# zju3dv/NeuralRecon-W

Measured on AMD Instinct MI355X. Metric: ray-samples/sec (train step) at 1024 rays x 128 samples, higher is better.
Workload: dtype f16; 1 GPU; brandenburg_gate config (BASELINE.json configs[1]): 1024 rays/GPU x (64 coarse + 64 fine) samples, SDF 8x256 + colour 4x256 + bg NeRF 8x256, 4 outside samples, up_sample_steps 2, render+loss+backward+allreduce+clip+Adam; rays_per_gpu=1024, samples_per_ray=128, global_rays=1024, parallelism=dp1, world_size=1, submission=eager, streams=2, skipped_steps=0

## Files before the change

neuralrecon-w_amd/csrc/ncw_color.hip:

```cpp
#include <stdlib.h>

#include "ncw_mlp.h"


namespace NCW_NS {

NCW_DEV void build_aux2(CVec<1>& aux, const float (&x)[3], const float (&nrm)[3], int lane) {
    const int h = lane >> 5;
#pragma unroll
    for (int r = 0; r < 16; ++r) {
        float v = 0.f;
        if (ncw_feat_of(r, 0) < 6) {
            const int f = ncw_feat_of(r, 0) + 4 * h;
            v = f == 0 ? x[0] : f == 1 ? x[1] : f == 2 ? x[2] : f == 3 ? nrm[0] : f == 4 ? nrm[1] : f == 5 ? nrm[2] : 0.f;
        }
        aux.v[0][r] = v;
    }
}

template <bool SPLIT, int RB_IN, int RB_OUT, int K_REAL, int SLOT, class P>
NCW_DEV void mma_stream_split(CVec<RB_OUT>& acc, const Act<P, RB_IN>& in, WRing& ring, const typename P::welem* __restrict__ w_hi,
                              const void* w_lo, int self_bytes, const void* w_next, int next_bytes, int lane) {
    typedef typename P::welem WE;
    if (SPLIT) {
// ... 19 lines not shown
        for (int r = 0; r < 16; ++r) yv[r] = ncw_relu(acc.v[rb][r]);
        if (st) stash_store_block(st, tile, RB, rb, yv, lane);
        to_act_block_hl<P, RB>(act, act_lo, rb, yv);
    }
}

template <int RB_IN, int RB_OUT, int K_REAL, int SLOT, class P>
NCW_DEV void mma_stream_split3(CVec<RB_OUT>& acc, const Act<P, RB_IN>& in, const Act<P, RB_IN>& in_lo, WRing& ring,
                               const typename P::welem* __restrict__ w_hi, const void* w_lo, int self_bytes, const void* w_next,
                               int next_bytes, int lane) {
    typedef typename P::welem WE;
    mma_stream2<RB_IN, RB_OUT, K_REAL, SLOT>(acc, in, in_lo, ring, w_hi, w_lo, self_bytes, lane);
    mma_stream<RB_IN, RB_OUT, K_REAL, SLOT>(acc, in, ring, (const WE*)w_lo, w_next, next_bytes, lane);
}

template <class P, int RBF, int RBH, int RBC, bool WIDE = false>
struct ColShapes {
    static constexpr int OCC = (RBF >= 16 || WIDE) ? 1 : 2;
    static constexpr int SLOT = RingSlot<RBC, OCC>::bytes;
    static constexpr int FCB_F = ncw_first_chunk_bytes<P, RBF, 32 * RBF, RBF, SLOT>();
    static constexpr int FCB_E0 = ncw_first_chunk_bytes<P, RBF + 3, 32 * RBF + 96, RBH, SLOT>();
    static constexpr int FCB_E = ncw_first_chunk_bytes<P, RBH, 32 * RBH, RBH, SLOT>();
    static constexpr int FCB_L0 = ncw_first_chunk_bytes<P, RBH + 1, 32 * RBH + 6, RBC, SLOT>();
    static constexpr int FCB_L = ncw_first_chunk_bytes<P, RBC, 32 * RBC, RBC, SLOT>();
    static constexpr int FCB_LAST = ncw_first_chunk_bytes<P, RBC, 32 * RBC, 1, SLOT>();
    static constexpr int FCB_TLAST = ncw_first_chunk_bytes<P, 1, 3, RBC, SLOT>();
    static constexpr int FCB_TL0 = ncw_first_chunk_bytes<P, RBC, 32 * RBC, RBH + 1, SLOT>();
    static constexpr int FCB_TE0 = ncw_first_chunk_bytes<P, RBH, 32 * RBH, RBF + 3, SLOT>();
};

template <class P, int RBF, int RBH, int RBC, int SPLIT, bool TRAIN>
NCW_DEV void color_fwd_body(const NcwColorNet& net, const NcwPoints& src, int64_t n, const float* __restrict__ normals,
                            const float* __restrict__ a, const void* __restrict__ feat_stash, float* __restrict__ rgb,
                            const NcwColorStash& st) {
    typedef typename P::welem WE;
    typedef typename P::selem SE;
    auto stp = [](void* p) -> SE* { return TRAIN ? (SE*)p : nullptr; };
    typedef ColShapes<P, RBF, RBH, RBC, SPLIT == 2> SH;
    constexpr bool AS = SPLIT == 2;
    NCW_RING_DECL(SH::SLOT);
    const int lane = ncw_lane();
    ring_prologue(ring, net.w_f, SH::FCB_F);
    int64_t tile, p, ray;
    bool valid;
    tile_setup(n, tile, p, valid, lane);
    float xs[3];
    load_point(src, p, xs, ray);
    const float dir[3] = {src.rays_d[ray * 3 + 0], src.rays_d[ray * 3 + 1], src.rays_d[ray * 3 + 2]};
    const float nrm[3] = {normals[p * 3 + 0], normals[p * 3 + 1], normals[p * 3 + 2]};

    Act<P, 3> aux1a;
    {
        CVec<3> aux1;
        build_aux1<Fast<P>::v>(aux1, dir, a + ray * net.n_a, net.n_a, lane);
        if (TRAIN) stash_store<3>((SE*)st.aux1, tile, aux1, lane);
        to_act(aux1a, aux1);
        if (st.aux_bias != nullptr) ncw_act_zero3(aux1a);
    }
    Act<P, 1> aux2a, aux2lo;
    {
        CVec<1> aux2;
        build_aux2(aux2, xs, nrm, lane);
        if (TRAIN) stash_store<1>((SE*)st.aux2, tile, aux2, lane);
        if constexpr (SPLIT != 0) {
#pragma unroll
            for (int t = 0; t < 2; ++t) ncw_split8(aux2.v[0], t, aux2a.f[t], aux2lo.f[t]);
        } else {
            to_act(aux2a, aux2);
        }
    }
    Act<P, RBF + 3> cat1;
    Act<P, (AS ? RBF + 3 : 1)> cat1_lo;
    {
        Act<P, RBF> fin;
#pragma unroll
        for (int rb = 0; rb < RBF; ++rb) {
            f32x16 v;
            stash_load_block(v, (const SE*)feat_stash, tile, RBF, rb, lane);
            to_act_block<RBF>(fin, rb, v);
        }
        CVec<RBF> f;
        load_bias(f, net.b_f, lane);
        mma_stream_split<(SPLIT != 0), RBF, RBF, 32 * RBF, SH::SLOT>(f, fin, ring, (const WE*)net.w_f, net.w_f_lo, SH::FCB_F, net.w_e[0],
                                                                SH::FCB_E0, lane);
        if (TRAIN) stash_store<RBF>((SE*)st.f, tile, f, lane);
        if constexpr (AS) {
            Act<P, RBF> fa, fl;
#pragma unroll
            for (int rb = 0; rb < RBF; ++rb) to_act_block_hl<P, RBF>(fa, fl, rb, f.v[rb]);
            act_concat<RBF, 3>(cat1, fa, aux1a);
            Act<P, 3> z3;
            ncw_act_zero3(z3);
            act_concat<RBF, 3>(cat1_lo, fl, z3);
        } else {
            Act<P, RBF> fa;
            to_act(fa, f);
            act_concat<RBF, 3>(cat1, fa, aux1a);
        }
    }
    Act<P, RBH> ea;
    Act<P, (AS ? RBH : 1)> ea_lo;
    {
        CVec<RBH> e;
        load_bias(e, net.b_e[0], lane);
        if (st.aux_bias != nullptr) ncw_add_ray_bias<RBH>(e, st.aux_bias + ray * (32 * RBH), lane);
        const void* wn = net.n_head > 1 ? net.w_e[1] : net.w_l[0];
        const int nb = net.n_head > 1 ? SH::FCB_E : SH::FCB_L0;
// ... 51 lines not shown
                mma_stream<RBH + 1, RBC, 32 * RBH + 6, SH::SLOT>(x, cat2, ring, (const WE*)net.w_l[0], net.w_l[1], nxt, lane);
            }
        } else {
            mma_stream_split<false, RBH + 1, RBC, 32 * RBH + 6, SH::SLOT>(x, cat2, ring, (const WE*)net.w_l[0], net.w_l_lo[0], SH::FCB_L0,
                                                                          net.w_l[1], 1 == last ? SH::FCB_LAST : SH::FCB_L, lane);
        }
        if constexpr (AS) relu_epilogue_hl<P, RBC>(xa, xa_lo, x, stp(st.x[0]), tile, lane);
        else relu_epilogue<P, RBC>(xa, x, stp(st.x[0]), tile, lane);
    }
    for (int l = 1; l < last; ++l) {
        load_bias(x, net.b_l[l], lane);
        if constexpr (AS) {
            mma_stream_split3<RBC, RBC, 32 * RBC, SH::SLOT>(x, xa, xa_lo, ring, (const WE*)net.w_l[l], net.w_l_lo[l], SH::FCB_L,
                                                            net.w_l[l + 1], l + 1 == last ? SH::FCB_LAST : SH::FCB_L, lane);
            relu_epilogue_hl<P, RBC>(xa, xa_lo, x, stp(st.x[l]), tile, lane);
        } else {
            mma_stream_split<(SPLIT != 0), RBC, RBC, 32 * RBC, SH::SLOT>(x, xa, ring, (const WE*)net.w_l[l], net.w_l_lo[l], SH::FCB_L,
                                                                    net.w_l[l + 1], l + 1 == last ? SH::FCB_LAST : SH::FCB_L, lane);
            relu_epilogue<P, RBC>(xa, x, stp(st.x[l]), tile, lane);
        }
    }
    CVec<1> o;
    load_bias(o, net.b_l[last], lane);
    if constexpr (AS)
        mma_stream_split3<RBC, 1, 32 * RBC, SH::SLOT>(o, xa, xa_lo, ring, (const WE*)net.w_l[last], net.w_l_lo[last], SH::FCB_LAST,
                                                      nullptr, 0, lane);
    else
        mma_stream_split<(SPLIT != 0), RBC, 1, 32 * RBC, SH::SLOT>(o, xa, ring, (const WE*)net.w_l[last], net.w_l_lo[last], SH::FCB_LAST,
                                                              nullptr, 0, lane);
    if (valid && lane < 32) {
        rgb[p * 3 + 0] = sigmoidf_<Fast<P>::v>(o.v[0][0]);
        rgb[p * 3 + 1] = sigmoidf_<Fast<P>::v>(o.v[0][1]);
        rgb[p * 3 + 2] = sigmoidf_<Fast<P>::v>(o.v[0][2]);
    }
}

template <class P, int RBF, int RBH, int RBC, int SPLIT = 0>
__global__ __launch_bounds__(64 * NCW_WG_WAVES, ((RBF >= 16 || SPLIT == 2) ? 1 : 2)) void color_fwd_kernel(NcwColorNet net, NcwPoints src, int64_t n,
                                                                      const float* __restrict__ normals,
                                                                      const float* __restrict__ a,
                                                                      const void* __restrict__ feat_stash,
                                                                      float* __restrict__ rgb, NcwColorStash st) {
    color_fwd_body<P, RBF, RBH, RBC, SPLIT, true>(net, src, n, normals, a, feat_stash, rgb, st);
}
template <class P, int RBF, int RBH, int RBC, int SPLIT = 0>
__global__ __launch_bounds__(64 * NCW_WG_WAVES, ((RBF >= 16 || SPLIT == 2) ? 1 : 2)) void color_render_kernel(NcwColorNet net, NcwPoints src, int64_t n,
                                                                         const float* __restrict__ normals,
                                                                         const float* __restrict__ a,
                                                                         const void* __restrict__ feat_stash,
                                                                         float* __restrict__ rgb, NcwColorStash st) {
    color_fwd_body<P, RBF, RBH, RBC, SPLIT, false>(net, src, n, normals, a, feat_stash, rgb, st);
}

template <class P, int RBF, int RBH, int RBC>
__global__ __launch_bounds__(64 * NCW_WG_WAVES, (RBF >= 16 ? 1 : 2)) void color_bwd_kernel(NcwColorNet net, NcwPoints src, int64_t n,
                                                                      const float* __restrict__ rgb,
                                                                      const float* __restrict__ d_rgb,
                                                                      float* __restrict__ d_grad, float* __restrict__ d_a,
                                                                      float* __restrict__ d_a_rows,
                                                                      void* __restrict__ dfeat_stash, NcwColorStash st) {
    typedef typename P::welem WE;
    typedef typename P::selem SE;
    typedef ColShapes<P, RBF, RBH, RBC> SH;
    NCW_RING_DECL(SH::SLOT);
    const int lane = ncw_lane();
    const int last = net.n_lin - 1;
    ring_prologue(ring, net.wt_l[last], SH::FCB_TLAST);
    int64_t tile, p, ray;
    bool valid;
    tile_setup(n, tile, p, valid, lane);
    ray = (src.mode == 0) ? p : p / src.per_ray;
    const float vm = valid ? 1.f : 0.f;

    CVec<1> zo;
    cvec_zero(zo);
    if (lane < 32) {
#pragma unroll
        for (int c = 0; c < 3; ++c) {
            const float y = rgb[p * 3 + c];
            zo.v[0][c] = d_rgb[p * 3 + c] * y * (1.f - y) * vm;
        }
    }
    stash_store<1>((SE*)st.zo, tile, zo, lane);
    Act<P, 1> zoa;
    to_act(zoa, zo);
    CVec<RBC> u;
    cvec_zero(u);
    mma_stream<1, RBC, 3, SH::SLOT>(u, zoa, ring, (const WE*)net.wt_l[last], net.wt_l[last - 1],
                                    last - 1 == 0 ? SH::FCB_TL0 : SH::FCB_L, lane);
    Act<P, RBC> za;
    for (int l = last - 1; l >= 1; --l) {
        relu_backward<P, RBC>(za, u, (const SE*)st.x[l], (SE*)st.zx[l], tile, lane);
        cvec_zero(u);
        mma_stream<RBC, RBC, 32 * RBC, SH::SLOT>(u, za, ring, (const WE*)net.wt_l[l], net.wt_l[l - 1],
                                                  l - 1 == 0 ? SH::FCB_TL0 : SH::FCB_L, lane);
    }
    CVec<RBH> ue;
    {
        relu_backward<P, RBC>(za, u, (const SE*)st.x[0], (SE*)st.zx[0], tile, lane);
        CVec<RBH + 1> q;
        cvec_zero(q);
        const void* wn = net.n_head > 1 ? net.wt_e[net.n_head - 1] : net.wt_e[0];
        const int nb = net.n_head > 1 ? SH::FCB_E : SH::FCB_TE0;
        mma_stream<RBC, RBH + 1, 32 * RBC, SH::SLOT>(q, za, ring, (const WE*)net.wt_l[0], wn, nb, lane);
#pragma unroll
        for (int rb = 0; rb < RBH; ++rb) ue.v[rb] = q.v[rb];
        if (valid) {
            if (lane < 32) d_grad[p * 3 + 0] += q.v[RBH][3];
            else {
                d_grad[p * 3 + 1] += q.v[RBH][0];
                d_grad[p * 3 + 2] += q.v[RBH][1];
            }
        }
    }
    Act<P, RBH> zea;
    for (int i = net.n_head - 1; i >= 1; --i) {
        relu_backward<P, RBH>(zea, ue, (const SE*)st.e[i], (SE*)st.ze[i], tile, lane);
        cvec_zero(ue);
        mma_stream<RBH, RBH, 32 * RBH, SH::SLOT>(ue, zea, ring, (const WE*)net.wt_e[i], net.wt_e[i - 1],
                                                  i - 1 == 0 ? SH::FCB_TE0 : SH::FCB_E, lane);
    }
    {
        relu_backward<P, RBH>(zea, ue, (const SE*)st.e[0], (SE*)st.ze[0], tile, lane);
        CVec<RBF + 3> q;
        cvec_zero(q);
        mma_stream<RBH, RBF + 3, 32 * RBH, SH::SLOT>(q, zea, ring, (const WE*)net.wt_e[0], net.wt_f, SH::FCB_F, lane);
        CVec<3> qa;
        qa.v[0] = q.v[RBF]; qa.v[1] = q.v[RBF + 1]; qa.v[2] = q.v[RBF + 2];
        accumulate_d_a(qa, d_a, ray, net.n_a, valid, lane, d_a_rows, p);
        CVec<RBF> zf;
#pragma unroll
        for (int rb = 0; rb < RBF; ++rb) zf.v[rb] = q.v[rb];
        stash_store<RBF>((SE*)st.zf, tile, zf, lane);
        Act<P, RBF> zfa;
        to_act(zfa, zf);
        CVec<RBF> df;
        cvec_zero(df);
        mma_stream<RBF, RBF, 32 * RBF, SH::SLOT>(df, zfa, ring, (const WE*)net.wt_f, nullptr, 0, lane);
        stash_store<RBF>((SE*)dfeat_stash, tile, df, lane);
    }
}

}
using namespace NCW_NS;

static bool color_ok(const NcwColorNet* net) {
    return net && net->n_head >= 1 && net->n_head <= 4 && net->n_lin >= 2 && net->n_lin <= 8 && net->n_a >= 0 &&
           net->n_a <= 69;
}

#define NCW_COLOR_DISPATCH(KERNEL, ...)                                                                          \
    do {                                                                                                         \
        const int key = net->rbf * 10000 + net->rbh * 100 + net->rbc;                                            \
        if (prec == NCW_PREC_F32) {                                                                              \
            if (key == 20102) NCW_LAUNCH_TILES((KERNEL<PrecF32, 2, 1, 2>), n, st, __VA_ARGS__);                  \
            else if (key == 20408) NCW_LAUNCH_TILES((KERNEL<PrecF32, 2, 4, 8>), n, st, __VA_ARGS__);             \
            else if (key == 80408) NCW_LAUNCH_TILES((KERNEL<PrecF32, 8, 4, 8>), n, st, __VA_ARGS__);             \
            else if (key == 160408) NCW_LAUNCH_TILES((KERNEL<PrecF32, 16, 4, 8>), n, st, __VA_ARGS__);           \
            else return NCW_E_UNSUPPORTED;                                                                       \
        } else {                                                                                                 \
            if (key == 20102) NCW_LAUNCH_TILES((KERNEL<PrecBF16, 2, 1, 2>), n, st, __VA_ARGS__);                 \
            else if (key == 20408) NCW_LAUNCH_TILES((KERNEL<PrecBF16, 2, 4, 8>), n, st, __VA_ARGS__);            \
            else if (key == 80408) NCW_LAUNCH_TILES((KERNEL<PrecBF16, 8, 4, 8>), n, st, __VA_ARGS__);            \
            else if (key == 160408) NCW_LAUNCH_TILES((KERNEL<PrecBF16, 16, 4, 8>), n, st, __VA_ARGS__);          \
            else return NCW_E_UNSUPPORTED;                                                                       \
        }                                                                                                        \
    } while (0)

#ifndef NCW_HALF_F16
extern "C" int ncw_color_fwd_f16(const NcwColorNet*, int, const NcwPoints*, int64_t, const float*, const float*, const void*, float*,
                                 const NcwColorStash*, void*);
extern "C" int ncw_color_bwd_f16(const NcwColorNet*, int, const NcwPoints*, int64_t, const float*, const float*, float*, float*, float*,
                                 void*, const NcwColorStash*, void*);
#endif

extern "C" int NCW_FN(ncw_color_fwd)(const NcwColorNet* net, int prec, const NcwPoints* pts, int64_t n, const float* normals,
                                     const float* a, const void* feat_stash, float* rgb, const NcwColorStash* stash,
                                     void* stream) {
    NCW_FORWARD_F16(prec, ncw_color_fwd_f16(net, NCW_PREC_BF16, pts, n, normals, a, feat_stash, rgb, stash, stream));
    if (!color_ok(net) || !pts || !stash || n < 0 || (prec != NCW_PREC_F32 && prec != NCW_PREC_BF16)) return NCW_E_BADARG;
    if (pts->mode == 4) return NCW_E_UNSUPPORTED;
    if (n == 0) return 0;
    hipStream_t st = (hipStream_t)stream;
    const bool render = stash->aux1 == nullptr;
    if (net->w_f_lo != nullptr) {
        if (prec == NCW_PREC_F32) return NCW_E_BADARG;
        const int key = net->rbf * 10000 + net->rbh * 100 + net->rbc;
        for (int i = 0; i < net->n_head; ++i) if (net->w_e_lo[i] == nullptr) return NCW_E_BADARG;
        for (int l = 0; l < net->n_lin; ++l) if (net->w_l_lo[l] == nullptr) return NCW_E_BADARG;
#define NCW_COLOR_SPLIT_DISPATCH(KERNEL, S)                                                                                               \
        do {                                                                                                                                    \
// ... 38 lines not shown
```

neuralrecon-w_amd/csrc/ncw_common.h:

```cpp
#pragma once
#include <hip/hip_runtime.h>
#include <stdint.h>
#include <type_traits>

#ifdef NCW_HALF_F16
typedef _Float16 ncw_h16;
#define NCW_MFMA_H __builtin_amdgcn_mfma_f32_32x32x16_f16
#define NCW_FN(name) name##_f16
#define NCW_NS ncw_h_f16
#else
typedef __bf16 ncw_h16;
#define NCW_MFMA_H __builtin_amdgcn_mfma_f32_32x32x16_bf16
#define NCW_FN(name) name
#define NCW_NS ncw_h_bf16
#endif
typedef ncw_h16 bf16x8 __attribute__((ext_vector_type(8)));
typedef ncw_h16 bf16x4 __attribute__((ext_vector_type(4)));
typedef float f32x16 __attribute__((ext_vector_type(16)));
typedef float f32x4 __attribute__((ext_vector_type(4)));

#define NCW_PREC_F32 0
#define NCW_PREC_BF16 1
#define NCW_PREC_F16 2
#ifdef NCW_HALF_F16
// ... 125 lines not shown
NCW_HD constexpr int ncw_chunk_units(int rb_stride, int n_units, int slot_bytes) {
    int g = slot_bytes / ncw_unit_bytes<P>(rb_stride);
    if (g < 1) g = 1;
    return g < n_units ? g : n_units;
}
template <class P, int RB_IN, int K_REAL, int RB_STRIDE, int SLOT>
NCW_HD constexpr int ncw_first_chunk_bytes() {
    return ncw_chunk_units<P>(RB_STRIDE, ncw_nb_used(RB_IN, K_REAL) * UnitsPerBlock<P>::v, SLOT) *
           ncw_unit_bytes<P>(RB_STRIDE);
}

NCW_DEV void ring_prologue(WRing& ring, const void* w_first, int first_bytes) {
    ring.cur = 0;
    ring_issue(ring.slot(0), w_first, first_bytes);
}

template <int RB_IN>
NCW_DEV float unit_b(const Act<PrecF32, RB_IN>& in, int rb, int sub) { return in.v[rb][sub]; }
template <int RB_IN>
NCW_DEV bf16x8 unit_b(const Act<PrecBF16, RB_IN>& in, int rb, int sub) { return in.f[2 * rb + sub]; }

NCW_DEV f32x16 unit_mfma(float a, float b, const f32x16& c) { return __builtin_amdgcn_mfma_f32_32x32x2f32(a, b, c, 0, 0, 0); }
NCW_DEV f32x16 unit_mfma(const bf16x8& a, const bf16x8& b, const f32x16& c) {
    return NCW_MFMA_H(a, b, c, 0, 0, 0);
}

template <class P>
NCW_HD constexpr int ncw_unit_first_feature(int rb, int sub) {
    return (P::id == NCW_PREC_F32) ? 32 * rb + ncw_feat_of(sub, 0) : 16 * (2 * rb + sub);
}

template <class P, int RB_IN_>
struct ActB {
    static constexpr int RB_IN = RB_IN_;
    const Act<P, RB_IN_>& a;
    NCW_DEV explicit ActB(const Act<P, RB_IN_>& a_) : a(a_) {}
    NCW_DEV void prepare(int) {}
    NCW_DEV auto b(int rb, int sub) const { return unit_b<RB_IN_>(a, rb, sub); }
};

template <class P, int RA, int RG>
struct CatB {
    static constexpr int RB_IN = RA + RG;
    const Act<P, RA>& a;
    const Act<P, RG>& g;
    NCW_DEV CatB(const Act<P, RA>& a_, const Act<P, RG>& g_) : a(a_), g(g_) {}
    NCW_DEV void prepare(int) {}
    NCW_DEV auto b(int rb, int sub) const {
        return rb < RA ? unit_b<RA>(a, rb < RA ? rb : 0, sub) : unit_b<RG>(g, rb >= RA ? rb - RA : 0, sub);
    }
};

struct NoB2 {};
template <int RB_OUT, int K_REAL, int SLOT, int RB_STRIDE, class P, class BP, bool PIPE = (SLOT != 32768) && (RB_OUT <= 8), class BP2 = NoB2>
NCW_DEV void mma_stream_b(CVec<RB_OUT>& acc, BP& bp, WRing& ring, const typename P::welem* __restrict__ wp,
                          const void* w_next, int next_bytes, int lane, BP2* bp2 = nullptr) {
    constexpr int RB_IN = BP::RB_IN;
    constexpr int UPB = UnitsPerBlock<P>::v;
    constexpr int NU = ncw_nb_used(RB_IN, K_REAL) * UPB;
    constexpr int UB = ncw_unit_bytes<P>(RB_STRIDE);
    constexpr int CU = ncw_chunk_units<P>(RB_STRIDE, NU, SLOT);
    constexpr int NCH = (NU + CU - 1) / CU;
    typedef typename std::conditional<P::id == NCW_PREC_F32, float, bf16x8>::type Frag;
#pragma unroll
    for (int c = 0; c < NCH; ++c) {
        __syncthreads();
        if (c + 1 < NCH) {
            const int nu = (c + 2) * CU <= NU ? CU : NU - (c + 1) * CU;
            ring_issue(ring.slot(ring.cur ^ 1), reinterpret_cast<const char*>(wp) + (size_t)(c + 1) * CU * UB, nu * UB);
        } else if (w_next != nullptr) {
            ring_issue(ring.slot(ring.cur ^ 1), w_next, next_bytes);
        }
        typedef const __attribute__((address_space(3))) Frag* lfrag_t;
        lfrag_t lw = (lfrag_t)(ring.slot(ring.cur)) + lane;
        Frag cur[RB_OUT], nxt[RB_OUT];
        bool loaded = false;
#pragma unroll
        for (int u = 0; u < CU; ++u) {
            const int q = c * CU + u;
            if (q >= NU) continue;
            const int rb = q / UPB, sub = q % UPB;
            if (sub == 0) bp.prepare(rb);
            if (ncw_unit_first_feature<P>(rb, sub) >= K_REAL) continue;
            if (!loaded) {
#pragma unroll
                for (int ro = 0; ro < RB_OUT; ++ro) cur[ro] = (lw + u * RB_STRIDE * 64)[ro * 64];
                loaded = true;
            }
            int un = -1;
#pragma unroll
            for (int v = CU - 1; v > u; --v) {
                const int qv = c * CU + v;
                if (qv < NU && ncw_unit_first_feature<P>(qv / UPB, qv % UPB) < K_REAL) un = v;
            }
            if (PIPE && un >= 0) {
#pragma unroll
                for (int ro = 0; ro < RB_OUT; ++ro) nxt[ro] = (lw + un * RB_STRIDE * 64)[ro * 64];
                __builtin_amdgcn_sched_barrier(0);
            }
            const auto b = bp.b(rb, sub);
#pragma unroll
            for (int ro = 0; ro < RB_OUT; ++ro) acc.v[ro] = unit_mfma(cur[ro], b, acc.v[ro]);
            if constexpr (!std::is_same<BP2, NoB2>::value) {
                const auto b2 = bp2->b(rb, sub);
#pragma unroll
                for (int ro = 0; ro < RB_OUT; ++ro) acc.v[ro] = unit_mfma(cur[ro], b2, acc.v[ro]);
            }
            if (PIPE && un >= 0) {
                __builtin_amdgcn_sched_barrier(0);
#pragma unroll
                for (int ro = 0; ro < RB_OUT; ++ro) cur[ro] = nxt[ro];
            } else {
                loaded = false;
                if (RB_OUT > 8) __builtin_amdgcn_sched_barrier(0);
            }
        }
        ring.cur ^= 1;
    }
}

template <int RB_IN, int RB_OUT, int K_REAL, int SLOT, int RB_STRIDE = RB_OUT, class P>
NCW_DEV void mma_stream(CVec<RB_OUT>& acc, const Act<P, RB_IN>& in, WRing& ring, const typename P::welem* __restrict__ wp,
                        const void* w_next, int next_bytes, int lane) {
    ActB<P, RB_IN> bp(in);
    mma_stream_b<RB_OUT, K_REAL, SLOT, RB_STRIDE, P>(acc, bp, ring, wp, w_next, next_bytes, lane);
}
template <int RB_IN, int RB_OUT, int K_REAL, int SLOT, int RB_STRIDE = RB_OUT, class P>
NCW_DEV void mma_stream2(CVec<RB_OUT>& acc, const Act<P, RB_IN>& in, const Act<P, RB_IN>& in2, WRing& ring,
                         const typename P::welem* __restrict__ wp, const void* w_next, int next_bytes, int lane) {
    ActB<P, RB_IN> bp(in), bp2(in2);
    mma_stream_b<RB_OUT, K_REAL, SLOT, RB_STRIDE, P, ActB<P, RB_IN>, (SLOT != 32768) && (RB_OUT <= 8), ActB<P, RB_IN>>(
        acc, bp, ring, wp, w_next, next_bytes, lane, &bp2);
}

template <int A, int B>
NCW_DEV void act_concat(Act<PrecF32, A + B>& o, const Act<PrecF32, A>& x, const Act<PrecF32, B>& y) {
#pragma unroll
    for (int i = 0; i < A; ++i) o.v[i] = x.v[i];
#pragma unroll
    for (int i = 0; i < B; ++i) o.v[A + i] = y.v[i];
}
template <int A, int B>
NCW_DEV void act_concat(Act<PrecBF16, A + B>& o, const Act<PrecBF16, A>& x, const Act<PrecBF16, B>& y) {
#pragma unroll
    for (int i = 0; i < 2 * A; ++i) o.f[i] = x.f[i];
#pragma unroll
    for (int i = 0; i < 2 * B; ++i) o.f[2 * A + i] = y.f[i];
}

NCW_HD constexpr size_t ncw_packed_elems(int rb_out, int rb_in) { return (size_t)rb_out * rb_in * 1024; }

template <int RB>
NCW_DEV void load_bias(CVec<RB>& acc, const float* __restrict__ bp, int lane) {
    const int h = lane >> 5;
#pragma unroll
    for (int rb = 0; rb < RB; ++rb) {
        const f32x4* b4 = reinterpret_cast<const f32x4*>(bp + (rb * 2 + h) * 16);
#pragma unroll
        for (int g = 0; g < 4; ++g) {
            f32x4 t = b4[g];
#pragma unroll
            for (int c = 0; c < 4; ++c) acc.v[rb][4 * g + c] = t[c];
        }
    }
}

NCW_DEV float ncw_relu(float x) {
    const int b = __builtin_bit_cast(int, x);
    return __builtin_bit_cast(float, b > 0 ? b : 0);
}

template <class V>
NCW_DEV V ncw_ld_frag(const void* w, size_t frag, int lane) {
    typedef const __attribute__((address_space(1))) V* gp;
    const char* base = (const char*)w + frag * (64 * sizeof(V));
    return *(gp)(base + (unsigned)lane * (unsigned)sizeof(V));
}

// ... 235 lines not shown
```

neuralrecon-w_amd/csrc/ncw_mlp.h:

```cpp
#pragma once
#include "../../include/neuconw_hip.h"
#include "ncw_common.h"

template <class P>
struct Fast { static constexpr bool v = (P::id == NCW_PREC_BF16); };

NCW_DEV void ncw_lds_barrier() {
    asm volatile("s_waitcnt lgkmcnt(0)" ::: "memory");
    __builtin_amdgcn_s_barrier();
    asm volatile("" ::: "memory");
}

NCW_DEV float grid_linspace(float start, float end, int steps, int i) {
    if (steps == 1) return start;
    const float step = (end - start) / (float)(steps - 1);
    return (i < steps / 2) ? start + step * (float)i : end - step * (float)(steps - 1 - i);
}

NCW_DEV int64_t points_count(const NcwPoints& s, int64_t n) {
    if (s.mode != 4) return n;
    const int64_t c = (int64_t)s.count[0];
    return c < n ? c : n;
}
NCW_DEV int64_t point_slot(const NcwPoints& s, int64_t p) { return s.mode == 4 ? (int64_t)s.idx[p] : p; }
// ... 210 lines not shown
    }
    NCW_DEV auto b(int rb, int sub) const {
        if constexpr (NX > 0) {
            if (rb >= RB) return unit_b<NX>(*extra, rb - RB, sub);
        }
        return unit_b<RB>(act, rb < RB ? rb : 0, sub);
    }
};

template <int RB>
NCW_DEV void cvec_copy(CVec<RB>& d, const CVec<RB>& s) {
#pragma unroll
    for (int i = 0; i < RB; ++i) d.v[i] = s.v[i];
}

#define NCW_WG_WAVES 4
#define NCW_LAUNCH_TILES(kernel, n, st, ...)                                                         \
    do {                                                                                            \
        const int64_t tiles__ = ((n) + 31) / 32;                                                    \
        const int64_t blocks__ = (tiles__ + NCW_WG_WAVES - 1) / NCW_WG_WAVES;                       \
        hipLaunchKernelGGL(kernel, dim3((unsigned)blocks__), dim3(64 * NCW_WG_WAVES), 0, st, __VA_ARGS__); \
        NCW_CHECK_LAUNCH();                                                                         \
    } while (0)

template <int RB, int OCC = 1>
struct RingSlot { static constexpr int bytes = RB >= 8 ? (OCC >= 2 ? 32768 : 65536) : 16384; };

#define NCW_RING_DECL(SLOTB)                                              \
    __shared__ __attribute__((aligned(16))) char ring_mem__[2 * (SLOTB)]; \
    WRing ring;                                                           \
    ring.base = (ncw_lchar*)ring_mem__;                                   \
    ring.cur = 0;                                                         \
    ring.slot_bytes = (SLOTB)

template <bool FAST>
NCW_DEV void build_aux1(CVec<3>& aux, const float (&dir)[3], const float* __restrict__ a_row, int n_a, int lane) {
    const int h = lane >> 5;
#pragma unroll
    for (int rb = 0; rb < 3; ++rb)
#pragma unroll
        for (int r = 0; r < 16; ++r) {
            const int f = 32 * rb + ncw_feat_of(r, 0) + 4 * h;
            float v;
            if (32 * rb + ncw_feat_of(r, 0) + 4 < 27) {
                v = freq_feature<3, 4, FAST>(dir, f);
            } else if (32 * rb + ncw_feat_of(r, 0) >= 27) {
                v = (f - 27 < n_a) ? a_row[f - 27] : 0.f;
            } else {
                v = (f < 27) ? freq_feature<3, 4, FAST>(dir, f) : ((f - 27 < n_a) ? a_row[f - 27] : 0.f);
            }
            aux.v[rb][r] = v;
        }
}

NCW_DEV void ncw_act_zero3(Act<PrecF32, 3>& a) {
#pragma unroll
    for (int i = 0; i < 3; ++i)
#pragma unroll
        for (int r = 0; r < 16; ++r) a.v[i][r] = 0.f;
}
NCW_DEV void ncw_act_zero3(Act<PrecBF16, 3>& a) {
#pragma unroll
    for (int i = 0; i < 6; ++i)
#pragma unroll
        for (int e = 0; e < 8; ++e) a.f[i][e] = (ncw_h16)0.f;
}
NCW_DEV void ncw_add_ray_bias_block(f32x16& v, const float* __restrict__ row, int rb, int lane) {
    const f32x4* ab = reinterpret_cast<const f32x4*>(row) + 8 * rb + (lane >> 5);
#pragma unroll
    for (int g = 0; g < 4; ++g) {
        const f32x4 t = ab[2 * g];
#pragma unroll
        for (int c = 0; c < 4; ++c) v[4 * g + c] += t[c];
    }
}
template <int RB>
NCW_DEV void ncw_add_ray_bias(CVec<RB>& e, const float* __restrict__ row, int lane) {
#pragma unroll
    for (int rb = 0; rb < RB; ++rb) ncw_add_ray_bias_block(e.v[rb], row, rb, lane);
}

NCW_DEV void accumulate_d_a(const CVec<3>& q, float* __restrict__ d_a, int64_t ray, int n_a, bool valid, int lane,
                            float* __restrict__ rows = nullptr, int64_t p = 0) {
    const int h = lane >> 5;
    if (rows != nullptr) {
#pragma unroll
        for (int rb = 0; rb < 3; ++rb)
#pragma unroll
            for (int r = 0; r < 16; ++r) {
                if (32 * rb + ncw_feat_of(r, 0) + 4 < 27) continue;
                const int j = 32 * rb + ncw_feat_of(r, 0) + 4 * h - 27;
                if (valid && j >= 0 && j < n_a) rows[p * n_a + j] = q.v[rb][r];
            }
        return;
    }
    const int64_t r0 = __shfl(ray, 0, 64);
    const bool uniform = __all((ray == r0) ? 1 : 0);
#pragma unroll
    for (int rb = 0; rb < 3; ++rb)
#pragma unroll
        for (int r = 0; r < 16; ++r) {
            if (32 * rb + ncw_feat_of(r, 0) + 4 < 27) continue;
            const int f = 32 * rb + ncw_feat_of(r, 0) + 4 * h;
            const int j = f - 27;
            float v = valid ? q.v[rb][r] : 0.f;
            if (uniform) {
// ... 9 lines not shown
```

neuralrecon-w_amd/csrc/ncw_nerf.hip:

```cpp
#include "ncw_mlp.h"

int NCW_FN(ncw_nerf_fwd8_launch)(const NcwNerfNet* net, const NcwPoints& src, const float* x4, int64_t n, const float* a, float* density,
                         float* rgb, const NcwNerfStash& stash, hipStream_t st);
int NCW_FN(ncw_nerf_bwd8_launch)(const NcwNerfNet* net, const NcwPoints& src, int64_t n, const float* d_density, const float* d_rgb,
                         float* d_a, const NcwNerfStash& stash, hipStream_t st);

namespace NCW_NS {

NCW_DEV void inverted_sphere(const float (&x)[3], float (&p4)[4]) {
    float r = sqrtf(x[0] * x[0] + x[1] * x[1] + x[2] * x[2]);
    r = fminf(fmaxf(r, 1.0f), 1e10f);
    p4[0] = x[0] / r; p4[1] = x[1] / r; p4[2] = x[2] / r; p4[3] = 1.0f / r;
}

template <class P, int RBN, int RBH, int OCC = 1>
struct NerfShapes {
    static constexpr int SLOT = RingSlot<RBN, OCC>::bytes;
    static constexpr int FCB_P0 = ncw_first_chunk_bytes<P, 3, 84, RBN, SLOT>();
    static constexpr int FCB_P = ncw_first_chunk_bytes<P, RBN, 32 * RBN, RBN, SLOT>();
    static constexpr int FCB_PS = ncw_first_chunk_bytes<P, RBN + 3, 32 * RBN + 84, RBN, SLOT>();
    static constexpr int FCB_ALPHA = ncw_first_chunk_bytes<P, RBN, 32 * RBN, 1, SLOT>();
    static constexpr int FCB_A0 = ncw_first_chunk_bytes<P, RBN + 3, 32 * RBN + 96, RBH, SLOT>();
    static constexpr int FCB_A = ncw_first_chunk_bytes<P, RBH, 32 * RBH, RBH, SLOT>();
    static constexpr int FCB_RGB = ncw_first_chunk_bytes<P, RBH, 32 * RBH, 1, SLOT>();
    static constexpr int FCB_TRGB = ncw_first_chunk_bytes<P, 1, 3, RBH, SLOT>();
    static constexpr int FCB_TA0 = ncw_first_chunk_bytes<P, RBH, 32 * RBH, RBN + 3, SLOT>();
    static constexpr int FCB_TALPHA = ncw_first_chunk_bytes<P, 1, 1, RBN, SLOT>();
    static constexpr int FCB_TPS = ncw_first_chunk_bytes<P, RBN, 32 * RBN, RBN + 3, SLOT>();
};

template <class P, int RBN, int RBH, bool TRAIN>
NCW_DEV void nerf_fwd_body(const NcwNerfNet& net, const NcwPoints& src, const float* __restrict__ x4, int64_t n,
                           const float* __restrict__ a, float* __restrict__ density, float* __restrict__ rgb,
                           const NcwNerfStash& st) {
    typedef typename P::welem WE;
    typedef typename P::selem SE;
    auto stp = [](void* p) -> SE* { return TRAIN ? (SE*)p : nullptr; };
    typedef NerfShapes<P, RBN, RBH> SH;
    NCW_RING_DECL(SH::SLOT);
    const int lane = ncw_lane();
    n = points_count(src, n);
    if ((int64_t)blockIdx.x * (blockDim.x >> 6) * 32 >= n) return;
    ring_prologue(ring, net.w_p[0], SH::FCB_P0);
    int64_t tile, p, ray;
    bool valid;
    tile_setup(n, tile, p, valid, lane);
    const int64_t ps = point_slot(src, p);
    float p4[4];
    if (x4) {
        p4[0] = x4[p * 4 + 0]; p4[1] = x4[p * 4 + 1]; p4[2] = x4[p * 4 + 2]; p4[3] = x4[p * 4 + 3];
        ray = p;
    } else {
        float xs[3];
        load_point(src, p, xs, ray);
        inverted_sphere(xs, p4);
    }
    const float dir[3] = {src.rays_d[ray * 3 + 0], src.rays_d[ray * 3 + 1], src.rays_d[ray * 3 + 2]};

    Act<P, 3> gpa;
    {
        CVec<3> gp;
        freq_encode<3, 4, 10, Fast<P>::v>(gp, p4, lane);
        if (TRAIN) stash_store<3>((SE*)st.gp, tile, gp, lane);
        to_act(gpa, gp);
    }
    Act<P, 3> aux1a;
    {
        CVec<3> aux1;
        build_aux1<Fast<P>::v>(aux1, dir, a + ray * net.n_a, net.n_a, lane);
        if (TRAIN) stash_store<3>((SE*)st.aux1, tile, aux1, lane);
        to_act(aux1a, aux1);
        if (st.aux_bias != nullptr) ncw_act_zero3(aux1a);
    }
    auto next_trunk = [&](int i, const void*& w, int& bytes) {
        const int m = i + 1;
        if (m < net.D) {
            w = net.w_p[m];
            bytes = (m == net.skip + 1) ? SH::FCB_PS : SH::FCB_P;
        } else {
            w = net.w_alpha;
            bytes = SH::FCB_ALPHA;
        }
    };
    const void* wn;
    int nb;
    CVec<RBN> acc;
    Act<P, RBN> ha;
    load_bias(acc, net.b_p[0], lane);
    next_trunk(0, wn, nb);
    mma_stream<3, RBN, 84, SH::SLOT>(acc, gpa, ring, (const WE*)net.w_p[0], wn, nb, lane);
    relu_epilogue<P, RBN>(ha, acc, stp(st.h[1]), tile, lane);
    for (int i = 1; i < net.D; ++i) {
        load_bias(acc, net.b_p[i], lane);
        next_trunk(i, wn, nb);
        if (i == net.skip + 1) {
            Act<P, RBN + 3> cat;
            act_concat<RBN, 3>(cat, ha, gpa);
            mma_stream<RBN + 3, RBN, 32 * RBN + 84, SH::SLOT>(acc, cat, ring, (const WE*)net.w_p[i], wn, nb, lane);
        } else {
            mma_stream<RBN, RBN, 32 * RBN, SH::SLOT>(acc, ha, ring, (const WE*)net.w_p[i], wn, nb, lane);
        }
        relu_epilogue<P, RBN>(ha, acc, stp(st.h[i + 1]), tile, lane);
    }
    {
        CVec<1> o;
        load_bias(o, net.b_alpha, lane);
        mma_stream<RBN, 1, 32 * RBN, SH::SLOT>(o, ha, ring, (const WE*)net.w_alpha, net.w_feat, SH::FCB_P, lane);
        if (valid && lane < 32) density[ps] = o.v[0][0];
    }
    Act<P, RBN + 3> cat1;
    {
        load_bias(acc, net.b_feat, lane);
        mma_stream<RBN, RBN, 32 * RBN, SH::SLOT>(acc, ha, ring, (const WE*)net.w_feat, net.w_a[0], SH::FCB_A0, lane);
        if (TRAIN) stash_store<RBN>((SE*)st.featn, tile, acc, lane);
        Act<P, RBN> fa;
        to_act(fa, acc);
        act_concat<RBN, 3>(cat1, fa, aux1a);
    }
    CVec<RBH> e;
    Act<P, RBH> ea;
    {
        load_bias(e, net.b_a[0], lane);
// ... 205 lines not shown
```

neuralrecon-w_amd/csrc/ncw_sdf8.hip:

```cpp
#include "ncw_mlp.h"

namespace {

constexpr int SB_WAVES = 8, SB_TILES = 4;

NCW_DEV void load_sprime_block_bf16(f32x16& sv, const ncw_h16* __restrict__ st_h, size_t tile, int RB, int rb, int lane) {
    stash_load_block(sv, st_h, tile, RB, rb, lane);
#pragma unroll
    for (int r = 0; r < 16; ++r) sv[r] = 1.f - __builtin_amdgcn_exp2f(sv[r] * -144.26950408889634f);
}
constexpr int SB_ACT = SB_TILES * 16 * 1024;
constexpr int SB_GAM = SB_TILES * 3 * 1024;

typedef __attribute__((address_space(3))) bf16x8 sb_lfrag;

template <int NU>
NCW_DEV void sb_load_slice(bf16x8* a, const void* w, int rb_stride, int ob, int u0, int lane) {
#pragma unroll
    for (int q = 0; q < NU; ++q) a[q] = ncw_ld_frag<bf16x8>(w, (size_t)(u0 + q) * rb_stride + ob, lane);
}

constexpr int SB_RD = 4;

template <int NU, bool TWO, int NPF = 0>
// ... 258 lines not shown
        const float s1 = x[1] * x[1], s2 = x[2] * x[2];
        r2 = __builtin_fmaf(x[0], x[0], s1) + s2;
    }
    float r = sqrtf(r2);
    r = fminf(fmaxf(r, 1.0f), 1e10f);
    p4[0] = x[0] / r; p4[1] = x[1] / r; p4[2] = x[2] / r; p4[3] = 1.0f / r;
}

template <bool TRAIN>
__global__ __launch_bounds__(64 * SB_WAVES) void nerf_fwdB_kernel(NcwNerfNet net, NcwPoints src, const float* __restrict__ x4,
                                                                 int64_t n, const float* __restrict__ a,
                                                                 float* __restrict__ density, float* __restrict__ rgb,
                                                                 NcwNerfStash st) {
    typedef ncw_h16 SE;
    __shared__ __attribute__((aligned(16))) char lds[2 * SB_ACT + SB_X + SB_TILES * 32 * 4];
    sb_lfrag* const abuf0 = (sb_lfrag*)(ncw_lchar*)lds;
    sb_lfrag* const abuf1 = abuf0 + SB_ACT / 16;
    sb_lfrag* const xbuf = abuf0 + 2 * SB_ACT / 16;
    typedef __attribute__((address_space(3))) int sb_lint;
    sb_lint* const rbuf = (sb_lint*)(xbuf + SB_X / 16);
    const int lane = ncw_lane();
    const int wave = __builtin_amdgcn_readfirstlane((int)(threadIdx.x >> 6));
    const int64_t tile0 = (int64_t)blockIdx.x * SB_TILES;
    const int D = net.D;
    n = points_count(src, n);
    if (tile0 * 32 >= n) return;
    int64_t pp = 0;
    bool pvalid = false;
    if (wave < SB_TILES) {
        int64_t p = (tile0 + wave) * 32 + (lane & 31), ray;
        pvalid = p < n;
        if (!pvalid) p = n - 1;
        pp = point_slot(src, p);
        float p4[4];
        if (x4) {
            p4[0] = x4[p * 4 + 0]; p4[1] = x4[p * 4 + 1]; p4[2] = x4[p * 4 + 2]; p4[3] = x4[p * 4 + 3];
            ray = p;
        } else {
            float xs[3];
            load_point(src, p, xs, ray);
            inverted_sphere8(xs, p4);
        }
        const float dir[3] = {src.rays_d[ray * 3 + 0], src.rays_d[ray * 3 + 1], src.rays_d[ray * 3 + 2]};
        if (lane < 32) rbuf[wave * 32 + lane] = (int)ray;
        CVec<3> gp;
        freq_encode<3, 4, 10, true>(gp, p4, lane);
        if (TRAIN) stash_store<3>((SE*)st.gp, (size_t)(tile0 + wave), gp, lane);
        Act<PrecBF16, 3> gpa;
        to_act(gpa, gp);
#pragma unroll
        for (int q = 0; q < 6; ++q) xbuf[(wave * 6 + q) * 64 + lane] = gpa.f[q];
        if (TRAIN) {
            CVec<3> aux1;
            build_aux1<true>(aux1, dir, a + ray * net.n_a, net.n_a, lane);
            stash_store<3>((SE*)st.aux1, (size_t)(tile0 + wave), aux1, lane);
        }
    }
    bf16x8 wa[16], wx[6];
    auto bias_of = [&](const float* bp, int ob) {
        CVec<1> b1;
        load_bias(b1, bp + ob * 32, lane);
        return b1.v[0];
    };
    auto relu16 = [](const f32x16& v) {
        f32x16 y;
#pragma unroll
        for (int r = 0; r < 16; ++r) y[r] = ncw_relu(v[r]);
        return y;
    };
    f32x16 bnext;
    {
        bf16x8 w0[6];
        const f32x16 bias = bias_of(net.b_p[0], wave);
        sb_load_slice<6>(w0, net.w_p[0], 8, wave, 0, lane);
        bnext = bias_of(D > 1 ? net.b_p[1] : net.b_feat, wave);
        sb_load_slice<16>(wa, D > 1 ? net.w_p[1] : net.w_feat, 8, wave, 0, lane);
        ncw_lds_barrier();
#pragma unroll
        for (int t = 0; t < SB_TILES; ++t) {
            f32x16 acc = bias;
            sb_mma<6, false>(acc, acc, w0, xbuf + t * 6 * 64 + lane, nullptr);
            const f32x16 y = relu16(acc);
            if (TRAIN) stash_store_block((SE*)st.h[1], (size_t)(tile0 + t), 8, wave, y, lane);
            sb_store_units(abuf0, t, wave, y, lane);
        }
    }
    int cur = 0;
    for (int i = 1; i < D; ++i) {
        const bool skip = (i == net.skip + 1);
        const void* wnext = i + 1 < D ? net.w_p[i + 1] : net.w_feat;
        const f32x16 bias = bnext;
        if (skip) sb_load_slice<6>(wx, net.w_p[i], 8, wave, 16, lane);
        bnext = bias_of(i + 1 < D ? net.b_p[i + 1] : net.b_feat, wave);
        ncw_lds_barrier();
        const sb_lfrag* in = cur ? abuf1 : abuf0;
        sb_lfrag* out = cur ? abuf0 : abuf1;
#pragma unroll
        for (int tp = 0; tp < SB_TILES; tp += 2) {
            f32x16 acc0 = bias, acc1 = bias;
            const sb_lfrag *in0 = in + tp * 16 * 64 + lane, *in1 = in0 + 16 * 64;
            if (tp == SB_TILES - 2) sb_mma<16, true, 16>(acc0, acc1, wa, in0, in1, wnext, 8, wave, lane);
            else sb_mma<16, true>(acc0, acc1, wa, in0, in1);
            if (skip) sb_mma<6, true>(acc0, acc1, wx, xbuf + tp * 6 * 64 + lane, xbuf + (tp + 1) * 6 * 64 + lane);
#pragma unroll
            for (int j = 0; j < 2; ++j) {
                const f32x16 y = relu16(j ? acc1 : acc0);
                if (TRAIN) stash_store_block((SE*)st.h[i + 1], (size_t)(tile0 + tp + j), 8, wave, y, lane);
                sb_store_units(out, tp + j, wave, y, lane);
            }
        }
        cur ^= 1;
    }
    const int hb = wave & 3, hp = wave >> 2;
    const int ta = 2 * hp, tb = 2 * hp + 1;
    {
        const f32x16 bias = bnext;
        ncw_lds_barrier();
        const sb_lfrag* in = cur ? abuf1 : abuf0;
        sb_lfrag* out = cur ? abuf0 : abuf1;
        if (wave < SB_TILES) {
            if (TRAIN || st.aux_bias == nullptr) {
                CVec<3> aux1;
                if (TRAIN) {
                    stash_load<3>(aux1, (const SE*)st.aux1, (size_t)(tile0 + wave), lane);
                } else {
                    const int64_t ray = rbuf[wave * 32 + (lane & 31)];
                    const float dir[3] = {src.rays_d[ray * 3 + 0], src.rays_d[ray * 3 + 1], src.rays_d[ray * 3 + 2]};
                    build_aux1<true>(aux1, dir, a + ray * net.n_a, net.n_a, lane);
                }
                Act<PrecBF16, 3> aux1a;
                to_act(aux1a, aux1);
#pragma unroll
                for (int q = 0; q < 6; ++q) xbuf[(wave * 6 + q) * 64 + lane] = aux1a.f[q];
            }
            __builtin_amdgcn_sched_barrier(0);
            bf16x8 w1[16];
            sb_load_slice<16>(w1, net.w_alpha, 1, 0, 0, lane);
            CVec<1> o;
            load_bias(o, net.b_alpha, lane);
            sb_mma<16, false>(o.v[0], o.v[0], w1, in + wave * 16 * 64 + lane, nullptr);
            if (pvalid && lane < 32) density[pp] = o.v[0][0];
        }
        sb_load_slice<6>(wx, net.w_a[0], 4, hb, 16, lane);
        bnext = bias_of(net.b_a[0], hb);
#pragma unroll
        for (int tp = 0; tp < SB_TILES; tp += 2) {
            f32x16 acc0 = bias, acc1 = bias;
            const sb_lfrag *in0 = in + tp * 16 * 64 + lane, *in1 = in0 + 16 * 64;
            if (tp == SB_TILES - 2) sb_mma<16, true, 16>(acc0, acc1, wa, in0, in1, net.w_a[0], 4, hb, lane);
            else sb_mma<16, true>(acc0, acc1, wa, in0, in1);
            if (TRAIN) {
                stash_store_block((SE*)st.featn, (size_t)(tile0 + tp), 8, wave, acc0, lane);
                stash_store_block((SE*)st.featn, (size_t)(tile0 + tp + 1), 8, wave, acc1, lane);
            }
            sb_store_units(out, tp, wave, acc0, lane);
            sb_store_units(out, tp + 1, wave, acc1, lane);
        }
        cur ^= 1;
    }
    for (int i = 0; i < net.n_head; ++i) {
        const bool more = i + 1 < net.n_head;
        const f32x16 bias = bnext;
        if (more) bnext = bias_of(net.b_a[i + 1], hb);
        f32x16 rb0, rb1;
        const bool ray_rows = (i == 0 && st.aux_bias != nullptr);
        if (ray_rows) {
            auto ray_row = [&](int t) {
                const f32x4* ab = reinterpret_cast<const f32x4*>(st.aux_bias + (size_t)rbuf[t * 32 + (lane & 31)] * 128) + 8 * hb + (lane >> 5);
                f32x16 v;
#pragma unroll
                for (int g = 0; g < 4; ++g) {
                    const f32x4 q = ab[2 * g];
#pragma unroll
                    for (int c = 0; c < 4; ++c) v[4 * g + c] = q[c];
                }
                return v;
            };
            rb0 = ray_row(ta);
            rb1 = ray_row(tb);
        }
        ncw_lds_barrier();
// ... 263 lines not shown
```

Measured before the change: 32.70 million ray-samples/s.

## Pipeline LDS weight fragment reads in color backward and batch aux1 appearance loads

Adds a read-ahead path to the streamed-weight MFMA loop. It keeps a small rotating set of LDS weight fragments loaded RD steps ahead of their MFMA use, and the color backward kernel now uses it for 16-bit precision with 8 feature blocks. Separately, a batched build_aux1 variant issues all appearance-embedding global loads up front before computing the frequency features, and it replaces the old version in the color, NeRF and SDF kernels. The aim is to hide LDS and global-load latency behind MFMA work, at the cost of more registers and sched_barriers that may limit compiler scheduling or occupancy.

```diff
diff --git a/neuralrecon-w_amd/csrc/ncw_color.hip b/neuralrecon-w_amd/csrc/ncw_color.hip
--- a/neuralrecon-w_amd/csrc/ncw_color.hip
+++ b/neuralrecon-w_amd/csrc/ncw_color.hip
@@ -95,7 +95,8 @@
     Act<P, 3> aux1a;
     {
         CVec<3> aux1;
-        build_aux1<Fast<P>::v>(aux1, dir, a + ray * net.n_a, net.n_a, lane);
+        if constexpr (P::id != NCW_PREC_F32 && RBF < 16) build_aux1_batched<Fast<P>::v>(aux1, dir, a + ray * net.n_a, net.n_a, lane);
+        else build_aux1<Fast<P>::v>(aux1, dir, a + ray * net.n_a, net.n_a, lane);
         if (TRAIN) stash_store<3>((SE*)st.aux1, tile, aux1, lane);
         to_act(aux1a, aux1);
         if (st.aux_bias != nullptr) ncw_act_zero3(aux1a);
@@ -253,6 +254,12 @@
     color_fwd_body<P, RBF, RBH, RBC, SPLIT, false>(net, src, n, normals, a, feat_stash, rgb, st);
 }
 
+#ifndef NCW_COLOR_BWD_RD
+#define NCW_COLOR_BWD_RD 3
+#endif
+#ifndef NCW_COLOR_BWD_RDW
+#define NCW_COLOR_BWD_RDW 2
+#endif
 template <class P, int RBF, int RBH, int RBC>
 __global__ __launch_bounds__(64 * NCW_WG_WAVES, (RBF >= 16 ? 1 : 2)) void color_bwd_kernel(NcwColorNet net, NcwPoints src, int64_t n,
                                                                       const float* __restrict__ rgb,
@@ -263,6 +270,8 @@
     typedef typename P::welem WE;
     typedef typename P::selem SE;
     typedef ColShapes<P, RBF, RBH, RBC> SH;
+    constexpr int RD = (P::id != NCW_PREC_F32 && RBF == 8) ? NCW_COLOR_BWD_RD : 0;
+    constexpr int RDW = RD < NCW_COLOR_BWD_RDW ? RD : NCW_COLOR_BWD_RDW;
     NCW_RING_DECL(SH::SLOT);
     const int lane = ncw_lane();
     const int last = net.n_lin - 1;
@@ -287,13 +296,13 @@
     to_act(zoa, zo);
     CVec<RBC> u;
     cvec_zero(u);
-    mma_stream<1, RBC, 3, SH::SLOT>(u, zoa, ring, (const WE*)net.wt_l[last], net.wt_l[last - 1],
+    mma_stream_rd<RD, 1, RBC, 3, SH::SLOT>(u, zoa, ring, (const WE*)net.wt_l[last], net.wt_l[last - 1],
                                     last - 1 == 0 ? SH::FCB_TL0 : SH::FCB_L, lane);
     Act<P, RBC> za;
     for (int l = last - 1; l >= 1; --l) {
         relu_backward<P, RBC>(za, u, (const SE*)st.x[l], (SE*)st.zx[l], tile, lane);
         cvec_zero(u);
-        mma_stream<RBC, RBC, 32 * RBC, SH::SLOT>(u, za, ring, (const WE*)net.wt_l[l], net.wt_l[l - 1],
+        mma_stream_rd<RD, RBC, RBC, 32 * RBC, SH::SLOT>(u, za, ring, (const WE*)net.wt_l[l], net.wt_l[l - 1],
                                                   l - 1 == 0 ? SH::FCB_TL0 : SH::FCB_L, lane);
     }
     CVec<RBH> ue;
@@ -303,7 +312,7 @@
         cvec_zero(q);
         const void* wn = net.n_head > 1 ? net.wt_e[net.n_head - 1] : net.wt_e[0];
         const int nb = net.n_head > 1 ? SH::FCB_E : SH::FCB_TE0;
-        mma_stream<RBC, RBH + 1, 32 * RBC, SH::SLOT>(q, za, ring, (const WE*)net.wt_l[0], wn, nb, lane);
+        mma_stream_rd<RD, RBC, RBH + 1, 32 * RBC, SH::SLOT>(q, za, ring, (const WE*)net.wt_l[0], wn, nb, lane);
 #pragma unroll
         for (int rb = 0; rb < RBH; ++rb) ue.v[rb] = q.v[rb];
         if (valid) {
@@ -318,14 +327,14 @@
     for (int i = net.n_head - 1; i >= 1; --i) {
         relu_backward<P, RBH>(zea, ue, (const SE*)st.e[i], (SE*)st.ze[i], tile, lane);
         cvec_zero(ue);
-        mma_stream<RBH, RBH, 32 * RBH, SH::SLOT>(ue, zea, ring, (const WE*)net.wt_e[i], net.wt_e[i - 1],
+        mma_stream_rd<RD, RBH, RBH, 32 * RBH, SH::SLOT>(ue, zea, ring, (const WE*)net.wt_e[i], net.wt_e[i - 1],
                                                   i - 1 == 0 ? SH::FCB_TE0 : SH::FCB_E, lane);
     }
     {
         relu_backward<P, RBH>(zea, ue, (const SE*)st.e[0], (SE*)st.ze[0], tile, lane);
         CVec<RBF + 3> q;
         cvec_zero(q);
-        mma_stream<RBH, RBF + 3, 32 * RBH, SH::SLOT>(q, zea, ring, (const WE*)net.wt_e[0], net.wt_f, SH::FCB_F, lane);
+        mma_stream_rd<RDW, RBH, RBF + 3, 32 * RBH, SH::SLOT>(q, zea, ring, (const WE*)net.wt_e[0], net.wt_f, SH::FCB_F, lane);
         CVec<3> qa;
         qa.v[0] = q.v[RBF]; qa.v[1] = q.v[RBF + 1]; qa.v[2] = q.v[RBF + 2];
         accumulate_d_a(qa, d_a, ray, net.n_a, valid, lane, d_a_rows, p);
@@ -337,7 +346,7 @@
         to_act(zfa, zf);
         CVec<RBF> df;
         cvec_zero(df);
-        mma_stream<RBF, RBF, 32 * RBF, SH::SLOT>(df, zfa, ring, (const WE*)net.wt_f, nullptr, 0, lane);
+        mma_stream_rd<RD, RBF, RBF, 32 * RBF, SH::SLOT>(df, zfa, ring, (const WE*)net.wt_f, nullptr, 0, lane);
         stash_store<RBF>((SE*)dfeat_stash, tile, df, lane);
     }
 }
diff --git a/neuralrecon-w_amd/csrc/ncw_common.h b/neuralrecon-w_amd/csrc/ncw_common.h
--- a/neuralrecon-w_amd/csrc/ncw_common.h
+++ b/neuralrecon-w_amd/csrc/ncw_common.h
@@ -201,7 +201,8 @@
 };
 
 struct NoB2 {};
-template <int RB_OUT, int K_REAL, int SLOT, int RB_STRIDE, class P, class BP, bool PIPE = (SLOT != 32768) && (RB_OUT <= 8), class BP2 = NoB2>
+template <int RB_OUT, int K_REAL, int SLOT, int RB_STRIDE, class P, class BP, bool PIPE = (SLOT != 32768) && (RB_OUT <= 8), class BP2 = NoB2,
+          int RD = 0>
 NCW_DEV void mma_stream_b(CVec<RB_OUT>& acc, BP& bp, WRing& ring, const typename P::welem* __restrict__ wp,
                           const void* w_next, int next_bytes, int lane, BP2* bp2 = nullptr) {
     constexpr int RB_IN = BP::RB_IN;
@@ -222,6 +223,34 @@
         }
         typedef const __attribute__((address_space(3))) Frag* lfrag_t;
         lfrag_t lw = (lfrag_t)(ring.slot(ring.cur)) + lane;
+        if constexpr (RD > 0) {
+            static_assert(P::id != NCW_PREC_F32 && std::is_same<BP2, NoB2>::value, "fragment ring: 16-bit, one B provider");
+            constexpr int QA = (K_REAL + 15) / 16 < NU ? (K_REAL + 15) / 16 : NU;
+            const int nau = QA - c * CU < 0 ? 0 : (QA - c * CU < CU ? QA - c * CU : CU);
+            const int nf = nau * RB_OUT;
+            Frag fr[RD];
+#pragma unroll
+            for (int i = 0; i < RD; ++i)
+                if (i < nf) fr[i] = (lw + (i / RB_OUT) * RB_STRIDE * 64)[(i % RB_OUT) * 64];
+#pragma unroll
+            for (int u = 0; u < CU; ++u) {
+                const int q = c * CU + u;
+                if (q >= NU) continue;
+                const int rb = q / UPB, sub = q % UPB;
+                if (sub == 0) bp.prepare(rb);
+                if (u >= nau) continue;
+                const auto b = bp.b(rb, sub);
+#pragma unroll
+                for (int ro = 0; ro < RB_OUT; ++ro) {
+                    const int i = u * RB_OUT + ro, j = i + RD;
+                    acc.v[ro] = unit_mfma(fr[i % RD], b, acc.v[ro]);
+                    if (j < nf) fr[i % RD] = (lw + (j / RB_OUT) * RB_STRIDE * 64)[(j % RB_OUT) * 64];
+                    __builtin_amdgcn_sched_barrier(0);
+                }
+            }
+            ring.cur ^= 1;
+            continue;
+        }
         Frag cur[RB_OUT], nxt[RB_OUT];
         bool loaded = false;
 #pragma unroll
@@ -273,6 +302,13 @@
                         const void* w_next, int next_bytes, int lane) {
     ActB<P, RB_IN> bp(in);
     mma_stream_b<RB_OUT, K_REAL, SLOT, RB_STRIDE, P>(acc, bp, ring, wp, w_next, next_bytes, lane);
+}
+template <int RD, int RB_IN, int RB_OUT, int K_REAL, int SLOT, class P>
+NCW_DEV void mma_stream_rd(CVec<RB_OUT>& acc, const Act<P, RB_IN>& in, WRing& ring, const typename P::welem* __restrict__ wp,
+                           const void* w_next, int next_bytes, int lane) {
+    ActB<P, RB_IN> bp(in);
+    mma_stream_b<RB_OUT, K_REAL, SLOT, RB_OUT, P, ActB<P, RB_IN>, (SLOT != 32768) && (RB_OUT <= 8), NoB2, RD>(acc, bp, ring, wp, w_next,
+                                                                                                          next_bytes, lane);
 }
 template <int RB_IN, int RB_OUT, int K_REAL, int SLOT, int RB_STRIDE = RB_OUT, class P>
 NCW_DEV void mma_stream2(CVec<RB_OUT>& acc, const Act<P, RB_IN>& in, const Act<P, RB_IN>& in2, WRing& ring,
diff --git a/neuralrecon-w_amd/csrc/ncw_mlp.h b/neuralrecon-w_amd/csrc/ncw_mlp.h
--- a/neuralrecon-w_amd/csrc/ncw_mlp.h
+++ b/neuralrecon-w_amd/csrc/ncw_mlp.h
@@ -286,6 +286,41 @@
             aux.v[rb][r] = v;
         }
 }
+template <bool FAST>
+NCW_DEV void build_aux1_batched(CVec<3>& aux, const float (&dir)[3], const float* __restrict__ a_row, int n_a, int lane) {
+    const int h = lane >> 5;
+    float av[3][16];
+    if (n_a > 0) {
+#pragma unroll
+        for (int rb = 0; rb < 3; ++rb)
+#pragma unroll
+            for (int r = 0; r < 16; ++r) {
+                if (32 * rb + ncw_feat_of(r, 0) + 4 < 27) continue;
+                const int j = 32 * rb + ncw_feat_of(r, 0) + 4 * h - 27;
+                av[rb][r] = a_row[j < 0 ? 0 : (j < n_a ? j : n_a - 1)];
+            }
+    } else {
+#pragma unroll
+        for (int rb = 0; rb < 3; ++rb)
+#pragma unroll
+            for (int r = 0; r < 16; ++r) av[rb][r] = 0.f;
+    }
+#pragma unroll
+    for (int rb = 0; rb < 3; ++rb)
+#pragma unroll
+        for (int r = 0; r < 16; ++r) {
+            const int f = 32 * rb + ncw_feat_of(r, 0) + 4 * h;
+            float v;
+            if (32 * rb + ncw_feat_of(r, 0) + 4 < 27) {
+                v = freq_feature<3, 4, FAST>(dir, f);
+            } else if (32 * rb + ncw_feat_of(r, 0) >= 27) {
+                v = (f - 27 < n_a) ? av[rb][r] : 0.f;
+            } else {
+                v = (f < 27) ? freq_feature<3, 4, FAST>(dir, f) : ((f - 27 < n_a) ? av[rb][r] : 0.f);
+            }
+            aux.v[rb][r] = v;
+        }
+}
 
 NCW_DEV void ncw_act_zero3(Act<PrecF32, 3>& a) {
 #pragma unroll
diff --git a/neuralrecon-w_amd/csrc/ncw_nerf.hip b/neuralrecon-w_amd/csrc/ncw_nerf.hip
--- a/neuralrecon-w_amd/csrc/ncw_nerf.hip
+++ b/neuralrecon-w_amd/csrc/ncw_nerf.hip
@@ -67,7 +67,8 @@
     Act<P, 3> aux1a;
     {
         CVec<3> aux1;
-        build_aux1<Fast<P>::v>(aux1, dir, a + ray * net.n_a, net.n_a, lane);
+        if constexpr (P::id != NCW_PREC_F32) build_aux1_batched<Fast<P>::v>(aux1, dir, a + ray * net.n_a, net.n_a, lane);
+        else build_aux1<Fast<P>::v>(aux1, dir, a + ray * net.n_a, net.n_a, lane);
         if (TRAIN) stash_store<3>((SE*)st.aux1, tile, aux1, lane);
         to_act(aux1a, aux1);
         if (st.aux_bias != nullptr) ncw_act_zero3(aux1a);
diff --git a/neuralrecon-w_amd/csrc/ncw_sdf8.hip b/neuralrecon-w_amd/csrc/ncw_sdf8.hip
--- a/neuralrecon-w_amd/csrc/ncw_sdf8.hip
+++ b/neuralrecon-w_amd/csrc/ncw_sdf8.hip
@@ -334,7 +334,7 @@
         for (int q = 0; q < 6; ++q) xbuf[(wave * 6 + q) * 64 + lane] = gpa.f[q];
         if (TRAIN) {
             CVec<3> aux1;
-            build_aux1<true>(aux1, dir, a + ray * net.n_a, net.n_a, lane);
+            build_aux1_batched<true>(aux1, dir, a + ray * net.n_a, net.n_a, lane);
             stash_store<3>((SE*)st.aux1, (size_t)(tile0 + wave), aux1, lane);
         }
     }
@@ -408,7 +408,7 @@
                 } else {
                     const int64_t ray = rbuf[wave * 32 + (lane & 31)];
                     const float dir[3] = {src.rays_d[ray * 3 + 0], src.rays_d[ray * 3 + 1], src.rays_d[ray * 3 + 2]};
-                    build_aux1<true>(aux1, dir, a + ray * net.n_a, net.n_a, lane);
+                    build_aux1_batched<true>(aux1, dir, a + ray * net.n_a, net.n_a, lane);
                 }
                 Act<PrecBF16, 3> aux1a;
                 to_act(aux1a, aux1);
```

New measurement: 32.79 million ray-samples/s, median of 6. About the same (+0.3%).
